# yaoyongxin/dmft-ed

Measured on AMD Instinct MI355X. Metric: Lanczos SpMV GB/s + ground-state iters/s, Ns=16 half-filled sector, 1/2/4/8 GPU, higher is better.
Workload: dtype f64; 1 GPU; c2: Norb=1 Nbath=7 (Nlevels=16) half-filled (4,4) sector, dim 4900, stored real(8) H, plain Lanczos 512 iters/step, persistent MODE 4 (4 = stored matrix in the Kronecker register layout); parallelism=sector replicas x1

## Files before the change

### dmft-ed_amd/csrc/ed_persist.hpp

```cpp
#pragma once
#include "ed_kernels.hpp"

namespace edg {

constexpr int kPBlock = 1024;
constexpr int kPChunk = 8;
constexpr int kPRegBlock = 512;

template <bool HC>
struct PersistRun {
  using H = val_t<HC>;
  const H* diag;
  const int64_t* sptr;
  const int32_t* cols;
  const H* vals;
  KronArgs<HC> K;
  int64_t dim;
  void* R;
  void* P;
  LancState* st;
  double* alpha;
  double* beta;
  void* basis;
  const uint32_t* pk;
  const H* dict;
  int ndict;
  const int32_t* kupc;
  const double* kupv;
  const int32_t* kdwc;
  const double* kdwv;
  const double* kdiag;
  int kdu, kdd, kdegu, kdegd;
  double thresh;
  int niter;
  int first;
  int64_t ldr, ldp;
  int64_t ldab;
};

template <int CTRL, int RM>
__device__ __forceinline__ double dpp_add(double v) {
  const int lo = __double2loint(v), hi = __double2hiint(v);
  const int l2 = __builtin_amdgcn_update_dpp(0, lo, CTRL, RM, 0xF, false);
  const int h2 = __builtin_amdgcn_update_dpp(0, hi, CTRL, RM, 0xF, false);
  return v + __hiloint2double(h2, l2);
}
__device__ __forceinline__ double wave_sum_dpp(double v) {
  v = dpp_add<0xB1, 0xF>(v);
  v = dpp_add<0x4E, 0xF>(v);
  v = dpp_add<0x141, 0xF>(v);
  v = dpp_add<0x140, 0xF>(v);
  v = dpp_add<0x142, 0xA>(v);
  v = dpp_add<0x143, 0xC>(v);
  return v;
}

template <int NT = kPBlock, bool TAIL = true>
__device__ __forceinline__ double pblock_sum(double v, double* ws) {
  v = wave_sum_dpp(v);
  if ((threadIdx.x & 63) == 63) ws[threadIdx.x >> 6] = v;
  __syncthreads();
  double t = 0.0;
#pragma unroll
  for (int w = 0; w < NT / 64; w++) t = t + ws[w];
  if constexpr (TAIL) __syncthreads();
  return t;
}

constexpr uint32_t kPkColBits = 17, kPkColMask = (1u << kPkColBits) - 1;
constexpr uint32_t kPkOffMask = (1u << 14) - 1;

__device__ __forceinline__ uint32_t lds_addr_of(const void* p) {
  return (uint32_t)(uintptr_t)(const __attribute__((address_space(3))) void*)p;
}
template <typename T>
__device__ __forceinline__ T lds_ldv(uint32_t a) {
  if constexpr (sizeof(T) == 16) {
    typedef double d2v __attribute__((ext_vector_type(2)));
    const d2v v = *(const __attribute__((address_space(3))) d2v*)(uintptr_t)a;
    return T{v.x, v.y};
  } else {
    return *(const __attribute__((address_space(3))) T*)(uintptr_t)a;
  }
}

struct PRows {
  int row0, stride, nvalid, iu;
};

template <int MODE, int RPT, int NT>
__device__ __forceinline__ PRows persist_rows(int tid, int64_t dim, int du, int dd) {
  PRows q;
  if constexpr (MODE == 4) {
    const int G = NT / du;
    if (tid < G * du) {
      const int g = tid / du;
      q.iu = tid - g * du;
      q.row0 = g * du + q.iu;
      q.stride = G * du;
      q.nvalid = dd > g ? (dd - g + G - 1) / G : 0;
    } else {
      q.iu = 0;
      q.row0 = G * du * RPT + (tid - G * du);
      q.stride = NT - G * du;
      q.nvalid = 0;
    }
  } else {
    q.iu = 0;
    q.row0 = tid;
    q.stride = NT;
    q.nvalid = dim > tid ? (int)((dim - tid + NT - 1) / NT) : 0;
  }
  return q;
}

template <bool HC, bool VC, int MODE, int RPT, int E = 1, int NT = kPBlock>
__global__ void __launch_bounds__(NT) k_lanc_persist(const PersistRun<HC> a) {
  using V = val_t<VC>;
  using H = val_t<HC>;
  extern __shared__ __align__(16) unsigned char smem[];
  __shared__ double ws[NT / 64];
  __shared__ double ws2[NT / 64];
  constexpr int VROWS = NT * RPT;
  constexpr bool SLOT = MODE == 4 && !VC;
  constexpr int VSLOT = NT + 1;
  constexpr int VLDS = SLOT ? RPT * VSLOT : VROWS;
  V* vl = (V*)smem;
  const int64_t dim = a.dim;
  const int tid = threadIdx.x;
  const int run = blockIdx.x;
  V* Rg = (V*)a.R + run * a.ldr;
  V* Pg = (V*)a.P + run * a.ldp;
  LancState* st = a.st + run;
  PRows q = persist_rows<MODE, RPT, NT>(tid, dim, a.kdu, a.kdd);
#define PROW(r) (q.row0 + (r) * q.stride)
#define LPOS(r) (SLOT ? (r) * VSLOT + tid : PROW(r))

  const H* aup = nullptr;
  const H* adw = nullptr;
  const H* upv = nullptr;
  const H* dwv = nullptr;
  const int32_t* upc = nullptr;
  const int32_t* dwc = nullptr;
  const uint8_t* impu = nullptr;
  const uint8_t* impd = nullptr;
  const double* uimp = nullptr;
  if constexpr (MODE == 1) {
    const KronArgs<HC>& K = a.K;
    unsigned char* qq = smem + (((int64_t)VROWS * sizeof(V) + 15) & ~(int64_t)15);
    auto carve = [&](int64_t bytes) {
      unsigned char* r = qq;
      qq += (bytes + 15) & ~(int64_t)15;
      return r;
    };
    H* s_aup = (H*)carve(K.dimup * sizeof(H));
    H* s_adw = (H*)carve(K.dimdw * sizeof(H));
    H* s_upv = (H*)carve((int64_t)K.degup * K.dimup * sizeof(H));
    H* s_dwv = (H*)carve((int64_t)K.degdw * K.dimdw * sizeof(H));
    int32_t* s_upc = (int32_t*)carve((int64_t)K.degup * K.dimup * 4);
    int32_t* s_dwc = (int32_t*)carve((int64_t)K.degdw * K.dimdw * 4);
    uint8_t* s_impu = (uint8_t*)carve(K.dimup);
    uint8_t* s_impd = (uint8_t*)carve(K.dimdw);
    double* s_uimp = (double*)carve((int64_t)K.nimp * K.nimp * 8);
    for (int64_t t = tid; t < K.dimup; t += NT) { s_aup[t] = K.aup[t]; s_impu[t] = K.impu[t]; }
    for (int64_t t = tid; t < K.dimdw; t += NT) { s_adw[t] = K.adw[t]; s_impd[t] = K.impd[t]; }
    for (int64_t t = tid; t < (int64_t)K.degup * K.dimup; t += NT) { s_upv[t] = K.upv[t]; s_upc[t] = K.upc[t]; }
    for (int64_t t = tid; t < (int64_t)K.degdw * K.dimdw; t += NT) { s_dwv[t] = K.dwv[t]; s_dwc[t] = K.dwc[t]; }
    for (int t = tid; t < K.nimp * K.nimp; t += NT) s_uimp[t] = K.uimp[t];
    aup = s_aup; adw = s_adw; upv = s_upv; dwv = s_dwv; upc = s_upc; dwc = s_dwc;
    impu = s_impu; impd = s_impd; uimp = s_uimp;
  }

  constexpr bool REG = MODE == 2 || MODE == 3;
  uint32_t pk[REG ? RPT * E : 1];
  const double* dg = nullptr;
  const unsigned char* dct = smem;
  if constexpr (MODE == 2) {
    const int64_t dbytes = ((int64_t)a.ndict * sizeof(H) + 15) & ~(int64_t)15;
    for (int t = tid; t < a.ndict; t += NT) ((H*)smem)[t] = a.dict[t];
    vl = (V*)(smem + dbytes);
    double* s_g = (double*)(smem + dbytes + (((int64_t)VROWS * sizeof(V) + 15) & ~(int64_t)15));
    for (int t = tid; t < VROWS; t += NT) s_g[t] = t < dim ? re_of(a.diag[t]) : 0.0;
    dg = s_g;
#pragma unroll
    for (int k = 0; k < RPT * E; k++) pk[k] = a.pk[k * NT + tid];
  }
  if constexpr (MODE == 3) {
    const KronArgs<HC>& K = a.K;
    const int du = (int)K.dimup, dd = (int)K.dimdw;
    const int nup = K.degup * du, ndw = K.degdw * dd;
    H* sd = (H*)smem;
    for (int t = tid; t < nup; t += NT) sd[t] = K.upv[t];
    for (int t = tid; t < ndw; t += NT) sd[nup + t] = K.dwv[t];
    if (tid == 0) sd[nup + ndw] = mk<HC>(0.0, 0.0);
    const int64_t dbytes = ((int64_t)(nup + ndw + 1) * sizeof(H) + 15) & ~(int64_t)15;
    vl = (V*)(smem + dbytes);
    double* s_g = (double*)(smem + dbytes + (((int64_t)VROWS * sizeof(V) + 15) & ~(int64_t)15));
    for (int t = tid; t < VROWS; t += NT) {
      const int iw = t / du, iu = t - iw * du;
      s_g[t] = t < dim ? re_of(add(add(K.aup[iu], K.adw[iw]), mk<HC>(K.uimp[K.impu[iu] * K.nimp + K.impd[iw]], 0.0)))
                       : 0.0;
    }
    dg = s_g;
    const uint32_t hs = sizeof(H);
    const uint32_t zero = (uint32_t)((nup + ndw) * hs) << kPkColBits;
#pragma unroll
    for (int r = 0; r < RPT; r++) {
      const int i = PROW(r);
      const int iw = i / du, iu = i - iw * du;
#pragma unroll
      for (int e = 0; e < E; e++) {
        uint32_t wd = zero;
        if (r < q.nvalid) {
          if (e < K.degup) {
            const int qq = e * du + iu;
            wd = (uint32_t)(iw * du + K.upc[qq]) | (((uint32_t)qq * hs) << kPkColBits);
          } else if (e < K.degup + K.degdw) {
            const int qq = (e - K.degup) * dd + iw;
            wd = (uint32_t)(K.dwc[qq] * du + iu) | (((uint32_t)(nup + qq) * hs) << kPkColBits);
          }
        }
        pk[r * E + e] = wd;
      }
    }
  }
  if constexpr (REG) {
    const uint32_t lbv = lds_addr_of(vl), lbd = lds_addr_of(dct);
#pragma unroll
    for (int k = 0; k < RPT * E; k++) {
      const uint32_t x = pk[k];
      pk[k] = (lbv + (x & kPkColMask) * (uint32_t)sizeof(V)) |
              ((lbd + ((x >> kPkColBits) & kPkOffMask)) << kPkColBits);
    }
  }
  constexpr bool KR = MODE == 4;
  constexpr bool KRC = KR && VC;
  uint32_t ucol[KR ? E : 1];
  double uval[KR ? E : 1];
  uint32_t dcol[KR ? RPT * E : 1];
  double dval[(KR && !VC) ? RPT * E : 1];
  double dgr[KR ? RPT : 1];
  const double* sdv = nullptr;
  int giw = 0;
  if constexpr (KR) {
    const int du = a.kdu, dd = a.kdd, G = NT / du;
    const bool act = tid < G * du;
    const int g = act ? tid / du : 0;
    giw = g;
    if constexpr (KRC) {
      double* t = (double*)(smem + (((int64_t)VLDS * sizeof(V) + 15) & ~(int64_t)15));
      for (int x = tid; x < E * dd; x += NT) t[x] = x < a.kdegd * dd ? a.kdwv[x] : 0.0;
      sdv = t;
    }
    const uint32_t lb = lds_addr_of(vl);
    constexpr uint32_t kLdsMask = (1u << 18) - 1;
#pragma unroll
    for (int e = 0; e < E; e++) {
      const bool ok = act && e < a.kdegu;
      if constexpr (SLOT) {
        const int pos = act ? g * du + (ok ? a.kupc[e * du + q.iu] : 0) : tid;
        ucol[e] = (lb + (uint32_t)pos * (uint32_t)sizeof(V)) & kLdsMask & ~(uint32_t)(sizeof(V) - 1);
      } else {
        ucol[e] = ok ? (uint32_t)a.kupc[e * du + q.iu] * (uint32_t)sizeof(V) : 0u;
      }
      uval[e] = ok ? a.kupv[e * du + q.iu] : 0.0;
    }
#pragma unroll
    for (int r = 0; r < RPT; r++) {
      const bool okr = r < q.nvalid;
      const int iw = g + G * r;
#pragma unroll
      for (int e = 0; e < E; e++) {
        const bool ok = okr && e < a.kdegd;
        int pos;
        if (ok) {
          const int iw2 = a.kdwc[e * dd + iw], r2 = iw2 / G;
          pos = SLOT ? r2 * VSLOT + (iw2 - r2 * G) * du + q.iu : iw2 * du + q.iu;
        } else {
          pos = okr ? 0 : LPOS(r);
        }
        dcol[r * E + e] = (SLOT ? lb : 0u) + (uint32_t)pos * (uint32_t)sizeof(V);
        if constexpr (!(KR && VC)) dval[r * E + e] = ok ? a.kdwv[e * dd + iw] : 0.0;
      }
      {
        double d = 0.0;
        if (okr) {
          if (a.kdiag) {
            d = a.kdiag[PROW(r)];
          } else {
            const KronArgs<HC>& K = a.K;
            d = re_of(add(add(K.aup[q.iu], K.adw[iw]), mk<HC>(K.uimp[K.impu[q.iu] * K.nimp + K.impd[iw]], 0.0)));
          }
        }
        dgr[r] = d;
      }
    }
  }

  constexpr bool PG = (REG || KRC) && VC;
  constexpr bool PIPE = KR && !VC && RPT * E <= 40;
  constexpr bool UREG = !VC && (REG || (KR && (!PIPE || RPT * E < 40)));
  V u[UREG ? RPT : 1];
  V p[PG ? 1 : RPT];
  uint32_t rix[RPT];
  double b, s;
  int it0;
  {
    double nrm = 0.0;
#pragma unroll
    for (int r = 0; r < RPT; r++) {
      const int i = PROW(r);
      const bool ok = r < q.nvalid;
      const V x = ok ? Rg[i] : vzero<V>();
      if constexpr (UREG) u[r] = x;
      vl[LPOS(r)] = x;
      if constexpr (!PG) p[r] = (ok && !a.first) ? Pg[i] : vzero<V>();
      if (a.first) {
        nrm += redot(x, x);
        if constexpr (PG) Pg[i] = vzero<V>();
      }
      if constexpr (MODE == 1) {
        const uint32_t w_ = (uint32_t)(i / a.K.dimup);
        rix[r] = ok ? (w_ << 16) | (uint32_t)(i - (int64_t)w_ * a.K.dimup) : 0u;
      }
    }
    if (a.first) {
      const double n2 = pblock_sum<NT>(nrm, ws);
      if (n2 == 0.0) {
        if (tid == 0) { st->iter = 0; st->done = 1; st->beta = 0.0; }
        return;
      }
      s = 1.0 / sqrt(n2);
      b = 0.0;
      it0 = 0;
      if (tid == 0) {
        st->iter = 0;
        st->done = 0;
        st->beta = 0.0;
      }
    } else {
      b = st->beta;
      s = 1.0 / b;
      it0 = st->iter;
    }
    __syncthreads();
  }
  if (st->done && !a.first) return;
  const double thresh = a.thresh;
  double* const alpha_out = a.alpha + run * a.ldab;
  double* const beta_out = a.beta + run * a.ldab;
  V* const basis = run == 0 ? (V*)a.basis : nullptr;

  for (int k = 0; k < a.niter; k++) {
    const int it = it0 + k;
    if constexpr (REG) {
#pragma unroll
      for (int e = 0; e < RPT * E; e++) asm volatile("" : "+v"(pk[e]));
    }
    if constexpr (KR) {
#pragma unroll
      for (int e = 0; e < RPT * E; e++) asm volatile("" : "+v"(dcol[e]));
    }
    asm volatile("" : "+v"(q.row0));
    V w[RPT];
    double ap = 0.0;
    if constexpr (PIPE) {
      double gu[E], gd[E], go;
      auto gather = [&](int r, double* hu, double* hd, double& ho) {
#pragma unroll
        for (int e = 0; e < E; e++) hu[e] = lds_ldv<double>(ucol[e] + r * VSLOT * 8);
#pragma unroll
        for (int e = 0; e < E; e++) hd[e] = lds_ldv<double>(dcol[r * E + e]);
        if constexpr (UREG) ho = u[r];
        else ho = vl[LPOS(r)];
      };
      gather(0, gu, gd, go);
#pragma unroll
      for (int r = 0; r < RPT; r++) {
        double nu[E], nd[E], no = 0.0;
        if (r + 1 < RPT) gather(r + 1, nu, nd, no);
        const double ur = go;
        double acc = ur * dgr[r];
#ifndef ED_P4_NOGATHER
#pragma unroll
        for (int e = 0; e < E; e++) acc = fma(uval[e], gu[e], acc);
#pragma unroll
        for (int e = 0; e < E; e++) acc = fma(dval[r * E + e], gd[e], acc);
#endif
        const double x = s * ur;
        w[r] = fma(s, acc, -(b * p[r]));
        ap = fma(x, w[r], ap);
        if (r + 1 < RPT) {
#pragma unroll
          for (int e = 0; e < E; e++) {
            gu[e] = nu[e];
            gd[e] = nd[e];
          }
          go = no;
        }
      }
    } else {
#pragma unroll
    for (int r = 0; r < RPT; r++) {
      const int i = PROW(r);
      const V ur = UREG ? u[r] : vl[LPOS(r)];
      V acc;
      if constexpr (MODE == 0) {
        acc = vzero<V>();
        if (r < q.nvalid) {
          const int64_t sl = i >> 6, s0 = a.sptr[sl];
          const int wd = (int)((a.sptr[sl + 1] - s0) >> 6);
          const int32_t* cp = a.cols + s0 + (i & 63);
          const H* vp = a.vals + s0 + (i & 63);
          acc = add(vzero<V>(), mul(a.diag[i], ur));
          for (int k0 = 0; k0 < wd; k0 += kPChunk) {
            int32_t c[kPChunk];
            H h[kPChunk];
#pragma unroll
            for (int kk = 0; kk < kPChunk; kk++) c[kk] = (k0 + kk < wd) ? cp[64 * (k0 + kk)] : 0;
#pragma unroll
            for (int kk = 0; kk < kPChunk; kk++)
              h[kk] = (k0 + kk < wd) ? vp[64 * (k0 + kk)] : mk<HC>(0.0, 0.0);
#pragma unroll
            for (int kk = 0; kk < kPChunk; kk++)
              if (k0 + kk < wd) acc = add(acc, mul(h[kk], vl[c[kk]]));
          }
        }
      } else if constexpr (REG) {
        acc = mul(dg[i], ur);
#pragma unroll
        for (int e = 0; e < E; e++) {
          const uint32_t x = pk[r * E + e];
          const H h = lds_ldv<H>(x >> kPkColBits);
          acc = fmac(acc, h, lds_ldv<V>(x & kPkColMask));
        }
      } else if constexpr (KR) {
        acc = mul(dgr[r], ur);
        {
        if constexpr (SLOT) {
#pragma unroll
          for (int e = 0; e < E; e++) acc = fmac(acc, uval[e], lds_ldv<V>(ucol[e] + r * VSLOT * (int)sizeof(V)));
        } else {
          const unsigned char* rb = (const unsigned char*)(vl + (i - q.iu));
#pragma unroll
          for (int e = 0; e < E; e++) acc = fmac(acc, uval[e], *(const V*)(rb + ucol[e]));
        }
        if constexpr (KR && VC) {
          const int iwc = min(giw + (NT / a.kdu) * r, a.kdd - 1);
#pragma unroll
          for (int e = 0; e < E; e++)
            acc = fmac(acc, sdv[e * a.kdd + iwc],
                       SLOT ? lds_ldv<V>(dcol[r * E + e]) : *(const V*)((const unsigned char*)vl + dcol[r * E + e]));
        } else {
#pragma unroll
          for (int e = 0; e < E; e++)
            acc = fmac(acc, dval[r * E + e], lds_ldv<V>(dcol[r * E + e]));
        }
        }
      } else {
        acc = vzero<V>();
        if (r < q.nvalid) {
          const int du = (int)a.K.dimup, dd = (int)a.K.dimdw;
          const int iwr = (int)(rix[r] >> 16), iur = (int)(rix[r] & 0xffffu);
          auto d = add(add(aup[iur], adw[iwr]), mk<HC>(uimp[impu[iur] * a.K.nimp + impd[iwr]], 0.0));
          acc = mul(d, ur);
          const V* xrow = vl + iwr * du;
          for (int kk = 0; kk < a.K.degup; kk++) {
            const int qq = kk * du + iur;
            acc = add(acc, mul(upv[qq], xrow[upc[qq]]));
          }
          for (int kk = 0; kk < a.K.degdw; kk++) {
            const int qq = kk * dd + iwr;
            acc = add(acc, mul(dwv[qq], vl[dwc[qq] * du + iur]));
          }
        }
      }
      const V x = scl(s, ur);
      V pr;
      if constexpr (PG) pr = Pg[i];
      else pr = p[r];
      w[r] = sub(scl(s, acc), scl(b, pr));
      ap += redot(x, w[r]);
    }
    }
#ifdef ED_P4_NOALPHA
    __syncthreads();
    const double alpha = ap * 1e-300;
#else
    const double alpha = pblock_sum<NT, false>(ap, ws);
#endif
    double bp = 0.0;
    if (basis) {
#pragma unroll
      for (int r = 0; r < RPT; r++)
        if (r < q.nvalid) basis[(int64_t)it * dim + PROW(r)] = scl(s, UREG ? u[r] : vl[LPOS(r)]);
    }
#pragma unroll
    for (int r = 0; r < RPT; r++) {
      const int i = PROW(r);
      const V x = scl(s, UREG ? u[r] : vl[LPOS(r)]);
      if constexpr (PIPE) {
        w[r] = fma(-alpha, x, w[r]);
        bp = fma(w[r], w[r], bp);
      } else {
        w[r] = sub(w[r], scl(alpha, x));
        bp += redot(w[r], w[r]);
      }
      if constexpr (PG) {
        Pg[i] = x;
      } else {
        p[r] = x;
      }
      if constexpr (UREG) u[r] = w[r];
      vl[LPOS(r)] = w[r];
    }
#ifdef ED_P4_NOBETA
    __syncthreads();
    const double bn = 1.0 + bp * 1e-300;
#else
    const double bn = sqrt(pblock_sum<NT, false>(bp, ws2));
#endif
    if (tid == 0) {
      alpha_out[it] = alpha;
      beta_out[it + 1] = bn;
    }
    b = bn;
    s = 1.0 / bn;
    if (bn < thresh) {
      if (tid == 0) {
        st->done = 1;
        st->iter = it + 1;
        st->beta = bn;
      }
      return;
    }
  }
#pragma unroll
  for (int r = 0; r < RPT; r++) {
    if (r < q.nvalid) {
      Rg[PROW(r)] = UREG ? u[r] : vl[LPOS(r)];
      if constexpr (!PG) Pg[PROW(r)] = p[r];
    }
  }
  if (tid == 0) {
    st->iter = it0 + a.niter;
    st->beta = b;
  }
#undef PROW
#undef LPOS
}

}
```

Baseline: 521,400 Lanczos iters/s.

## Prefetch next iteration's row-0 gather across beta reduction; reuse scaled vector

The first row's LDS gather for the next Lanczos iteration now starts right after the beta reduction and before the sqrt and store. This lets its latency overlap the iteration boundary instead of stalling at the top of the loop. In the pipelined path the scaled vector s*u is also computed once into p[r] and reused for the basis store and the alpha update, rather than recomputed. The DPP shuffles switch to mov_dpp with bound_ctrl. The changes add loop-carried register state and a scheduling barrier, which may raise register pressure.

New measurement: 583,700 Lanczos iters/s, median of 6. 11.9% higher.

```diff
diff --git a/dmft-ed_amd/csrc/ed_persist.hpp b/dmft-ed_amd/csrc/ed_persist.hpp
--- a/dmft-ed_amd/csrc/ed_persist.hpp
+++ b/dmft-ed_amd/csrc/ed_persist.hpp
@@ -41,8 +41,8 @@
 template <int CTRL, int RM>
 __device__ __forceinline__ double dpp_add(double v) {
   const int lo = __double2loint(v), hi = __double2hiint(v);
-  const int l2 = __builtin_amdgcn_update_dpp(0, lo, CTRL, RM, 0xF, false);
-  const int h2 = __builtin_amdgcn_update_dpp(0, hi, CTRL, RM, 0xF, false);
+  const int l2 = __builtin_amdgcn_mov_dpp(lo, CTRL, RM, 0xF, true);
+  const int h2 = __builtin_amdgcn_mov_dpp(hi, CTRL, RM, 0xF, true);
   return v + __hiloint2double(h2, l2);
 }
 __device__ __forceinline__ double wave_sum_dpp(double v) {
@@ -351,6 +351,19 @@
   double* const beta_out = a.beta + run * a.ldab;
   V* const basis = run == 0 ? (V*)a.basis : nullptr;
 
+  double gu[PIPE ? E : 1], gd[PIPE ? E : 1], go = 0.0;
+  auto gather = [&](int r, double* hu, double* hd, double& ho) {
+    if constexpr (PIPE) {
+#pragma unroll
+      for (int e = 0; e < E; e++) hu[e] = lds_ldv<double>(ucol[e] + r * VSLOT * 8);
+#pragma unroll
+      for (int e = 0; e < E; e++) hd[e] = lds_ldv<double>(dcol[r * E + e]);
+      if constexpr (UREG) ho = u[r];
+      else ho = vl[LPOS(r)];
+    }
+  };
+  gather(0, gu, gd, go);
+
   for (int k = 0; k < a.niter; k++) {
     const int it = it0 + k;
     if constexpr (REG) {
@@ -365,16 +378,6 @@
     V w[RPT];
     double ap = 0.0;
     if constexpr (PIPE) {
-      double gu[E], gd[E], go;
-      auto gather = [&](int r, double* hu, double* hd, double& ho) {
-#pragma unroll
-        for (int e = 0; e < E; e++) hu[e] = lds_ldv<double>(ucol[e] + r * VSLOT * 8);
-#pragma unroll
-        for (int e = 0; e < E; e++) hd[e] = lds_ldv<double>(dcol[r * E + e]);
-        if constexpr (UREG) ho = u[r];
-        else ho = vl[LPOS(r)];
-      };
-      gather(0, gu, gd, go);
 #pragma unroll
       for (int r = 0; r < RPT; r++) {
         double nu[E], nd[E], no = 0.0;
@@ -387,9 +390,11 @@
 #pragma unroll
         for (int e = 0; e < E; e++) acc = fma(dval[r * E + e], gd[e], acc);
 #endif
-        const double x = s * ur;
-        w[r] = fma(s, acc, -(b * p[r]));
-        ap = fma(x, w[r], ap);
+        double bpr = b * p[r];
+        asm volatile("" : "+v"(bpr));
+        p[r] = s * ur;
+        w[r] = fma(s, acc, -bpr);
+        ap = fma(p[r], w[r], ap);
         if (r + 1 < RPT) {
 #pragma unroll
           for (int e = 0; e < E; e++) {
@@ -493,12 +498,14 @@
     if (basis) {
 #pragma unroll
       for (int r = 0; r < RPT; r++)
-        if (r < q.nvalid) basis[(int64_t)it * dim + PROW(r)] = scl(s, UREG ? u[r] : vl[LPOS(r)]);
+        if (r < q.nvalid) basis[(int64_t)it * dim + PROW(r)] = PIPE ? p[r] : scl(s, UREG ? u[r] : vl[LPOS(r)]);
     }
 #pragma unroll
     for (int r = 0; r < RPT; r++) {
       const int i = PROW(r);
-      const V x = scl(s, UREG ? u[r] : vl[LPOS(r)]);
+      V x;
+      if constexpr (PIPE) x = p[r];
+      else x = scl(s, UREG ? u[r] : vl[LPOS(r)]);
       if constexpr (PIPE) {
         w[r] = fma(-alpha, x, w[r]);
         bp = fma(w[r], w[r], bp);
@@ -508,7 +515,7 @@
       }
       if constexpr (PG) {
         Pg[i] = x;
-      } else {
+      } else if constexpr (!PIPE) {
         p[r] = x;
       }
       if constexpr (UREG) u[r] = w[r];
@@ -516,9 +523,18 @@
     }
 #ifdef ED_P4_NOBETA
     __syncthreads();
-    const double bn = 1.0 + bp * 1e-300;
+    const double bsq = 1.0 + bp * 1e-300;
 #else
-    const double bn = sqrt(pblock_sum<NT, false>(bp, ws2));
+    const double bsq = pblock_sum<NT, false>(bp, ws2);
+#endif
+    if constexpr (PIPE) {
+      gather(0, gu, gd, go);
+      __builtin_amdgcn_sched_barrier(0);
+    }
+#ifdef ED_P4_NOBETA
+    const double bn = bsq;
+#else
+    const double bn = sqrt(bsq);
 #endif
     if (tid == 0) {
       alpha_out[it] = alpha;
```
